# Tangshitao/Semi-supervised-Adaptive-Distillation

Measured on AMD Instinct MI355X. Metric: images/sec (student+teacher fwd + student bwd) R50-FPN distill, 1/2/4/8 MI355X, higher is better.
Workload: dtype f32

## Files before the change

include/ssad_kernels.h:

```cpp
#ifndef SSAD_KERNELS_H_
#define SSAD_KERNELS_H_

#include <stddef.h>
#include <stdint.h>

#ifdef __cplusplus
extern "C" {
#endif

#define SSAD_API __attribute__((visibility("default")))

#define SSAD_E_BADARG (-1)
#define SSAD_E_WORKSPACE (-2)
#define SSAD_MAX_LEVELS 8
#define SSAD_MAX_CONV_PROBLEMS 24
#define SSAD_MAX_POWSUM_INPUTS 8

typedef void* ssad_stream_t;


typedef struct {
  float gamma;
  float alpha;
  float beta;
// ... 223 lines not shown
    const double* cell_anchors, int levels, int A, int k_min, const int* field_sizes_host,
    const int* crop_h_host, const int* crop_w_host, const float* gt_boxes,
    const int* gt_classes, const int* gt_counts, int N, int Gmax, int num_classes,
    float positive_overlap, float negative_overlap, int* const* labels_out_host,
    float* const* locs_out_host, float* const* targets_out_host, int capacity,
    int* counts_out, float* fg_bg_out, void* workspace, size_t workspace_bytes,
    ssad_stream_t stream, int class_specific_bbox);


#define SSAD_IMAGE_BLOBS_MAX_BATCH 64
typedef struct ssad_image_norm {
  float div, mean[3], std[3];
  float* out;
} ssad_image_norm;
SSAD_API size_t ssad_image_blobs_workspace_bytes(int N, int Hb, int Wb);
SSAD_API int ssad_image_blobs(
    const unsigned char* src, size_t src_bytes, const long long* offset_host, const int* h_host,
    const int* w_host, const int* out_h_host, const int* out_w_host, const double* scale_host,
    const int* flipped_host, int N, int Hb, int Wb, const ssad_image_norm* norms_host, int n_norms,
    void* workspace, size_t workspace_bytes, ssad_stream_t stream);


SSAD_API int ssad_conv_out_size(int in, int kernel, int dilation, int pad_a, int pad_b, int stride);
SSAD_API int ssad_im2col(const float* x, int C, int H, int W, int kh, int kw, int dil_h, int dil_w,
                         int pad_t, int pad_l, int pad_b, int pad_r, int stride_h, int stride_w,
                         float* col, ssad_stream_t stream);
SSAD_API int ssad_im2col_batched(const float* x, int N, int C, int H, int W, int kernel, int stride,
                                 int pad, float* col, ssad_stream_t stream);
SSAD_API int ssad_col2im(const float* col, int C, int H, int W, int kh, int kw, int dil_h,
                         int dil_w, int pad_t, int pad_l, int pad_b, int pad_r, int stride_h,
                         int stride_w, float* x, ssad_stream_t stream);
SSAD_API int ssad_channel_sum(const float* dy, int N, int C, int HW, float* out, int accumulate,
                              ssad_stream_t stream);
SSAD_API int ssad_relu_grad_rowsum(const float* y, const float* dy, float* dx, float* rowsum, int N,
                                   int C, int HW, ssad_stream_t stream);
SSAD_API int ssad_conv1x1_bias_act(const float* x, const float* w, const float* bias,
                                   const float* residual, float* y, int N, int C, int P, int M,
                                   int relu, ssad_stream_t stream);
SSAD_API int ssad_conv1x1_bias_act2(const float* x, int C1, const float* x2, int C2, const float* w,
                                    const float* bias, const float* residual, float* y, int N, int P,
                                    int M, int relu, ssad_stream_t stream);
#define SSAD_GEMM_RELU 1
#define SSAD_GEMM_ACCUMULATE 8
typedef struct ssad_gemm_conv {
  const float* a;
  const float* x;
  float* y;
  const float* bias;
  const float* residual;
  const float* mask;
  int lda, N, K, P, M, flags;
} ssad_gemm_conv;
SSAD_API int ssad_conv1x1_gemm(const ssad_gemm_conv* desc_host, ssad_stream_t stream);
SSAD_API size_t ssad_conv1x1_gemm_split_workspace_bytes(const ssad_gemm_conv* desc_host);
SSAD_API int ssad_conv1x1_gemm_split(const ssad_gemm_conv* desc_host, void* workspace, size_t workspace_bytes,
                                     ssad_stream_t stream);
SSAD_API int ssad_conv1x1_gemm_split_amax(const ssad_gemm_conv* desc_host, const float* packed_a, const unsigned* x_amax,
                                          unsigned* y_amax_out, void* workspace, size_t workspace_bytes,
                                          ssad_stream_t stream);
typedef struct ssad_gemm_pack_entry {
  const float* a;
  float* dst;
  int lda, K, M;
} ssad_gemm_pack_entry;
SSAD_API size_t ssad_gemm_split_filter_floats(int K, int M);
SSAD_API int ssad_gemm_split_pack_filters(const ssad_gemm_pack_entry* entries_host, int n_entries, ssad_stream_t stream);
SSAD_API int ssad_conv_implicit_gemm(const ssad_gemm_conv* d, int C, int H, int W, int kernel, int stride, int pad,
                                     ssad_stream_t stream);
SSAD_API size_t ssad_conv_implicit_gemm_workspace_bytes(int N, int M, int C, int H, int W, int kernel, int stride,
                                                        int pad);
SSAD_API int ssad_conv_implicit_gemm_ws(const ssad_gemm_conv* d, int C, int H, int W, int kernel, int stride, int pad,
                                        void* workspace, size_t workspace_bytes, ssad_stream_t stream);
SSAD_API size_t ssad_conv_kxk_wgrad_workspace_bytes(int N, int C, int H, int W, int M, int kernel, int stride,
                                                    int pad);
SSAD_API int ssad_conv_kxk_wgrad(const float* x, const float* dy, int N, int C, int H, int W, int M, int kernel,
                                 int stride, int pad, float* dw, int accumulate, void* workspace,
                                 size_t workspace_bytes, ssad_stream_t stream);
SSAD_API size_t ssad_conv_kxk_dgrad_workspace_bytes(int N, int C, int H, int W, int M, int kernel, int stride,
                                                    int pad);
SSAD_API int ssad_conv_kxk_dgrad(const float* w, const float* dy, int N, int C, int H, int W, int M, int kernel,
                                 int stride, int pad, float* dx, const float* mask, int accumulate, void* workspace,
                                 size_t workspace_bytes, ssad_stream_t stream);
SSAD_API int ssad_transpose_filter(const float* w, int M, int K, int ldm, float* wt, ssad_stream_t stream);
#define SSAD_MAX_TRANSPOSE_ENTRIES 64
typedef struct ssad_transpose_entry {
  const float* w;
  float* wt;
  int M, K, ldm;
  int reserved;
} ssad_transpose_entry;
SSAD_API int ssad_transpose_filters(const ssad_transpose_entry* entries_host, int n_entries, ssad_stream_t stream);
SSAD_API size_t ssad_conv1x1_wgrad_workspace_bytes(int N, int C, int P, int M);
SSAD_API int ssad_conv1x1_wgrad(const float* x, const float* dy, int N, int C, int P, int M, float* dw,
                                int accumulate, void* workspace, size_t workspace_bytes,
                                ssad_stream_t stream);
SSAD_API size_t ssad_conv1x1_wgrad_split_workspace_bytes(int N, int C, int P, int M);
SSAD_API int ssad_conv1x1_wgrad_split(const float* x, const float* dy, int N, int C, int P, int M, float* dw,
                                      int accumulate, void* workspace, size_t workspace_bytes,
                                      ssad_stream_t stream);
SSAD_API int ssad_conv1x1_wgrad_split_amax(const float* x, const float* dy, int N, int C, int P, int M, float* dw,
                                           int accumulate, void* workspace, size_t workspace_bytes,
                                           const unsigned* x_amax, const unsigned* dy_amax, ssad_stream_t stream);
SSAD_API int ssad_subsample(const float* x, int N, int C, int H, int W, int stride, float* y,
                            ssad_stream_t stream);
SSAD_API int ssad_subsample_grad(const float* dy, int N, int C, int H, int W, int stride, int accumulate,
                                 float* dx, ssad_stream_t stream);
// ... 277 lines not shown
```

semi-supervised-adaptive-distillation_amd/csrc/kernels/gemm_conv.hip:

```cpp
#include <hip/hip_runtime.h>
#include <stdint.h>
#include <stdlib.h>

#include "conv_internal.h"
#include "ssad_kernels.h"

namespace {

using ssad_dev::uniform_rsrc;
typedef float f32x16 __attribute__((ext_vector_type(16)));
typedef __attribute__((address_space(3))) void* lds_ptr;

constexpr int kThreads = 256;
constexpr unsigned kOob = 0x80000000u;
constexpr int BN = 128;
constexpr int BK = 16;
constexpr int NSTAGE = 3;

struct GemmArgs {
  const float* a;
  const float* x;
  float* y;
  const float* bias;
  const float* res;
  const float* mask;
  int lda, N, K, P, M, flags;
  int mtiles, ctiles;
  long long Q;
  int C, H, W, OW, ksize, stride, pad;
  int splits, per_split;
  float* part;
};

__device__ __forceinline__ float ldf(__amdgpu_buffer_rsrc_t rs, unsigned off) {
  return __builtin_bit_cast(float, __builtin_amdgcn_raw_buffer_load_b32(rs, off, 0, 0));
}
__device__ __forceinline__ void stf(float v, __amdgpu_buffer_rsrc_t rs, unsigned off) {
  __builtin_amdgcn_raw_buffer_store_b32(__builtin_bit_cast(unsigned, v), rs, off, 0, 0);
}

__device__ __forceinline__ int xcd_remap(int b, int total) {
  const int q = total >> 3, r = total & 7;
  const int xcd = b & 7, k = b >> 3;
  return (xcd < r ? xcd * (q + 1) : r * (q + 1) + (xcd - r) * q) + k;
}

template <int BM, bool IMPLICIT = false>
__global__ __launch_bounds__(kThreads, 3) void gemm_conv_nn_kernel(const GemmArgs g) {
  constexpr int TI = BM / 64;
  constexpr int A_STAGE = BK * BM;
  constexpr int B_STAGE = BK * BN;
  constexpr int STAGE = A_STAGE + B_STAGE;
  constexpr int A_ROW_LANES = BM / 4;
  constexpr int A_ROWS_PER_INSTR = 64 / A_ROW_LANES;
  constexpr int A_INSTR = BK / A_ROWS_PER_INSTR;
  constexpr int B_INSTR = BK / 2;
  constexpr int A_PER_WAVE = A_INSTR / 4;
  constexpr int B_PER_WAVE = IMPLICIT ? BK * (BN / 64) / 4 : B_INSTR / 4;
  constexpr int LOADS = A_PER_WAVE + B_PER_WAVE;
  __shared__ __attribute__((aligned(16))) float lds[NSTAGE * STAGE];

  const int tid = threadIdx.x, lane = tid & 63, wave = __builtin_amdgcn_readfirstlane(tid >> 6);
  const int wm = wave & 1, wn = wave >> 1;
  const int j = lane & 31, h = lane >> 5;
  const int ntiles = g.mtiles * g.ctiles;
  const int split = g.splits > 1 ? (int)blockIdx.x / ntiles : 0;
  const int tile = xcd_remap((int)blockIdx.x - split * ntiles, ntiles);
  const int mt = tile % g.mtiles, ct = tile / g.mtiles;
  const int m0 = mt * BM;
  const long long q0 = (long long)ct * BN;
  const int K = g.K, P = g.P;

  const __amdgpu_buffer_rsrc_t ars = uniform_rsrc(g.a, (unsigned)((long long)K * g.lda * 4));
  const __amdgpu_buffer_rsrc_t xrs = uniform_rsrc(
      g.x, IMPLICIT ? (unsigned)((long long)g.N * g.C * g.H * g.W * 4) : (unsigned)((long long)g.N * K * P * 4));

  const int a_row = lane / A_ROW_LANES, a_col = (lane % A_ROW_LANES) * 4;
  unsigned a_voff = (unsigned)((a_row * g.lda + m0 + a_col) * 4);
  if (m0 + a_col >= g.lda) a_voff = kOob;
  const long long qb = q0 + (lane & 31) * 4;
  unsigned b_voff = kOob;
  if (qb < g.Q) {
    const int n = (int)(qb / P), p = (int)(qb - (long long)n * P);
    b_voff = (unsigned)((((long long)n * K + h) * P + p) * 4);
  }
  int ioff[2] = {0, 0};
  unsigned ymask[2] = {0, 0}, xmask[2] = {0, 0};
  int s_c[4] = {0, 0, 0, 0}, s_ky[4] = {0, 0, 0, 0}, s_kx[4] = {0, 0, 0, 0};
  int d_c = 0, d_ky = 0, d_kx = 0;
  if (IMPLICIT) {
#pragma unroll
    for (int hf = 0; hf < 2; ++hf) {
      const long long qc = q0 + hf * 64 + lane;
      const bool ok = qc < g.Q;
      const int n = ok ? (int)(qc / P) : 0, pp = ok ? (int)(qc - (long long)n * P) : 0;
      const int iy0 = (pp / g.OW) * g.stride - g.pad, ix0 = (pp % g.OW) * g.stride - g.pad;
      ioff[hf] = ((n * g.C * g.H + iy0) * g.W + ix0) * 4;
      if (ok)
        for (int t = 0; t < g.ksize; ++t) {
          ymask[hf] |= (unsigned)((unsigned)(iy0 + t) < (unsigned)g.H) << t;
          xmask[hf] |= (unsigned)((unsigned)(ix0 + t) < (unsigned)g.W) << t;
        }
    }
    const int kk2 = g.ksize * g.ksize;
    const int row0 = (g.splits > 1 ? split * g.per_split : 0) * BK + wave * 4;
#pragma unroll
    for (int v = 0; v < 4; ++v) {
      const int row = row0 + v, c = row / kk2, r2 = row - c * kk2;
      s_c[v] = c; s_ky[v] = r2 / g.ksize; s_kx[v] = r2 - s_ky[v] * g.ksize;
    }
    d_c = BK / kk2;
    const int d_r = BK - d_c * kk2;
    d_ky = d_r / g.ksize; d_kx = d_r - d_ky * g.ksize;
  }
  auto issue = [&](int chunk, int buf) {
    const int k0 = chunk * BK;
    float* base = lds + buf * STAGE;
    const bool tail = k0 + BK > K;
#pragma unroll
    for (int u = 0; u < A_PER_WAVE; ++u) {
      const int ia = wave * A_PER_WAVE + u;
      const int row = k0 + ia * A_ROWS_PER_INSTR;
      unsigned vo = a_voff;
      if (tail) vo = (row + a_row < K) ? a_voff : kOob;
      __builtin_amdgcn_raw_ptr_buffer_load_lds(ars, (lds_ptr)(base + ia * 256), 16, vo, row * g.lda * 4, 0, 0);
    }
    if (IMPLICIT) {
#pragma unroll
      for (int u = 0; u < B_PER_WAVE; ++u) {
        const int ib = wave * B_PER_WAVE + u;
        const int rr = ib >> 1, hf = ib & 1, v = u >> 1;
        const int soff = ((s_c[v] * g.H + s_ky[v]) * g.W + s_kx[v]) * 4;
        const unsigned in = (ymask[hf] >> s_ky[v]) & (xmask[hf] >> s_kx[v]) & 1u;
        unsigned vo = in ? (unsigned)(ioff[hf] + soff) : kOob;
        if (tail) vo = (k0 + rr < K) ? vo : kOob;
        __builtin_amdgcn_raw_ptr_buffer_load_lds(xrs, (lds_ptr)(base + A_STAGE + rr * BN + hf * 64), 4, vo, 0, 0, 0);
      }
#pragma unroll
      for (int v = 0; v < 4; ++v) {
        s_kx[v] += d_kx;
        if (s_kx[v] >= g.ksize) { s_kx[v] -= g.ksize; ++s_ky[v]; }
        s_ky[v] += d_ky;
        if (s_ky[v] >= g.ksize) { s_ky[v] -= g.ksize; ++s_c[v]; }
        s_c[v] += d_c;
      }
    } else {
#pragma unroll
      for (int u = 0; u < B_PER_WAVE; ++u) {
        const int ib = wave * B_PER_WAVE + u;
        const int row = k0 + ib * 2;
        unsigned vo = b_voff;
        if (tail) vo = (row + h < K) ? b_voff : kOob;
        __builtin_amdgcn_raw_ptr_buffer_load_lds(xrs, (lds_ptr)(base + A_STAGE + ib * 256), 16, vo, row * P * 4, 0, 0);
      }
    }
  };

  f32x16 acc[TI][2];
#pragma unroll
  for (int i = 0; i < TI; ++i)
#pragma unroll
    for (int t = 0; t < 2; ++t)
#pragma unroll
      for (int r = 0; r < 16; ++r) acc[i][t][r] = 0.0f;

  int chunk0 = 0, chunks = (K + BK - 1) / BK;
  if (g.splits > 1) {
    chunk0 = split * g.per_split;
    chunks = chunks < chunk0 + g.per_split ? chunks : chunk0 + g.per_split;
  }
  issue(chunk0, 0);
  if (chunk0 + 1 < chunks) issue(chunk0 + 1, 1);
  const int a_rd = wm * (BM / 2) + j;
  const int b_rd = A_STAGE + wn * 64 + j;
  int buf = 0;
  for (int c = chunk0; c < chunks; ++c) {
    if (c + 1 < chunks) {
      asm volatile("s_waitcnt vmcnt(%0)" ::"n"(LOADS) : "memory");
    } else {
      asm volatile("s_waitcnt vmcnt(0)" ::: "memory");
    }
    __builtin_amdgcn_s_barrier();
    if (c + 2 < chunks) issue(c + 2, buf == 0 ? 2 : buf - 1);
    typedef const volatile __attribute__((address_space(3))) float* lds_cvf;
    const lds_cvf sa = (lds_cvf)(lds + buf * STAGE + a_rd + h * BM);
    const lds_cvf sb = (lds_cvf)(lds + buf * STAGE + b_rd + h * BN);
    float av[2][TI], bv[2][2];
#pragma unroll
    for (int i = 0; i < TI; ++i) av[0][i] = sa[i * 32];
#pragma unroll
    for (int t = 0; t < 2; ++t) bv[0][t] = sb[t * 32];
#pragma unroll
    for (int ks = 0; ks < BK / 2; ++ks) {
      const int cur = ks & 1, nxt = cur ^ 1;
      if (ks + 1 < BK / 2) {
        const int k = 2 * (ks + 1);
#pragma unroll
        for (int i = 0; i < TI; ++i) av[nxt][i] = sa[k * BM + i * 32];
#pragma unroll
        for (int t = 0; t < 2; ++t) bv[nxt][t] = sb[k * BN + t * 32];
      }
      __builtin_amdgcn_sched_barrier(0);
#pragma unroll
      for (int i = 0; i < TI; ++i)
#pragma unroll
        for (int t = 0; t < 2; ++t)
          acc[i][t] = __builtin_amdgcn_mfma_f32_32x32x2f32(av[cur][i], bv[cur][t], acc[i][t], 0, 0, 0);
      __builtin_amdgcn_sched_barrier(0);
    }
    if (++buf == NSTAGE) buf = 0;
  }

  const bool partial = g.splits > 1;
  const bool relu = !partial && (g.flags & SSAD_GEMM_RELU), accum = !partial && (g.flags & SSAD_GEMM_ACCUMULATE);
  const float* const gbias = partial ? nullptr : g.bias;
  const float* const gres = partial ? nullptr : g.res;
  const float* const gmask = partial ? nullptr : g.mask;
  const long long ybytes = (long long)g.N * g.M * P * 4;
  float* const yout = partial ? g.part + (long long)split * ((long long)g.N * g.M * P) : g.y;
  const __amdgpu_buffer_rsrc_t yrs = uniform_rsrc(yout, (unsigned)ybytes);
  const __amdgpu_buffer_rsrc_t rrs = uniform_rsrc(gres ? gres : yout, (unsigned)ybytes);
  const __amdgpu_buffer_rsrc_t krs = uniform_rsrc(gmask ? gmask : yout, (unsigned)ybytes);
#pragma unroll
  for (int i = 0; i < TI; ++i) {
    float bvv[16];
#pragma unroll
    for (int r = 0; r < 16; ++r) bvv[r] = 0.0f;
    if (gbias) {
#pragma unroll
      for (int r = 0; r < 16; ++r) {
        const int m = m0 + wm * (BM / 2) + i * 32 + (r & 3) + 8 * (r >> 2) + 4 * h;
        bvv[r] = gbias[m < g.M ? m : g.M - 1];
      }
    }
#pragma unroll
    for (int t = 0; t < 2; ++t) {
      const long long q = q0 + wn * 64 + t * 32 + j;
      long long col = -1;
      if (q < g.Q) {
        const int n = (int)(q / P), p = (int)(q - (long long)n * P);
        col = (long long)n * g.M * P + p;
      }
      unsigned off[16];
#pragma unroll
      for (int r = 0; r < 16; ++r) {
        const int m = m0 + wm * (BM / 2) + i * 32 + (r & 3) + 8 * (r >> 2) + 4 * h;
        off[r] = (col >= 0 && m < g.M) ? (unsigned)((col + (long long)m * P) * 4) : kOob;
      }
      f32x16 v = acc[i][t];
#pragma unroll
      for (int r = 0; r < 16; ++r) v[r] += bvv[r];
      if (gres) {
        float tmp[16];
#pragma unroll
        for (int r = 0; r < 16; ++r) tmp[r] = ldf(rrs, off[r]);
#pragma unroll
        for (int r = 0; r < 16; ++r) v[r] += tmp[r];
      }
      if (relu) {
#pragma unroll
        for (int r = 0; r < 16; ++r) v[r] = fmaxf(v[r], 0.0f);
      }
      if (gmask) {
        float tmp[16];
#pragma unroll
        for (int r = 0; r < 16; ++r) tmp[r] = ldf(krs, off[r]);
#pragma unroll
        for (int r = 0; r < 16; ++r) v[r] = tmp[r] > 0.0f ? v[r] : 0.0f;
      }
      if (accum) {
        float tmp[16];
#pragma unroll
        for (int r = 0; r < 16; ++r) tmp[r] = ldf(yrs, off[r]);
#pragma unroll
        for (int r = 0; r < 16; ++r) v[r] += tmp[r];
      }
#pragma unroll
      for (int r = 0; r < 16; ++r) stf(v[r], yrs, off[r]);
    }
  }
}

struct WgradArgs {
  const float* x;
  const float* dy;
  float* part;
  int N, C, P, M;
  int mtiles, ctiles;
  int chunks;
  int per_split;
  int splits;
  int xcd_group;
};

__global__ __launch_bounds__(kThreads, 3) void gemm_conv_nt_kernel(const WgradArgs g) {
  constexpr int TSTAGE = 128 * BK;
  constexpr int STAGE = 2 * TSTAGE;
  __shared__ __attribute__((aligned(16))) float lds[NSTAGE * STAGE];
  const int tid = threadIdx.x, lane = tid & 63, wave = __builtin_amdgcn_readfirstlane(tid >> 6);
  const int wm = wave & 1, wn = wave >> 1;
  const int j = lane & 31, h = lane >> 5;
  int v = (int)blockIdx.x;
  {
    const int G = (int)gridDim.x, xg = g.xcd_group;
    if (xg > 1 && (G & 7) == 0 && ((G >> 3) % xg) == 0) {
      const int r = v >> 3, x = v & 7;
      v = (r / xg) * (8 * xg) + x * xg + (r % xg);
    }
  }
  const int ntiles = g.mtiles * g.ctiles;
  const int split = v / ntiles, tile = v - split * ntiles;
  const int mt = tile % g.mtiles, ct = tile / g.mtiles;
  const int m0 = mt * 128, c0 = ct * 128;
  const int P = g.P;
  const int ch0 = split * g.per_split;
  const int ch1 = min(ch0 + g.per_split, g.chunks);
  const int nch = ch1 - ch0;

  const __amdgpu_buffer_rsrc_t yrs = uniform_rsrc(g.dy, (unsigned)((long long)g.N * g.M * P * 4));
  const __amdgpu_buffer_rsrc_t xrs = uniform_rsrc(g.x, (unsigned)((long long)g.N * g.C * P * 4));

  const int d_row = lane >> 2, d_slot = lane & 3;
  unsigned vy0[2], vx0[2];
#pragma unroll
  for (int u = 0; u < 2; ++u) {
    const int row = (wave * 2 + u) * 16 + d_row;
    const int piece = d_slot ^ ((row >> 2) & 3);
    vy0[u] = (m0 + row < g.M) ? (unsigned)((((long long)(m0 + row)) * P + piece * 4) * 4) : kOob;
    vx0[u] = (c0 + row < g.C) ? (unsigned)((((long long)(c0 + row)) * P + piece * 4) * 4) : kOob;
  }
  auto issue = [&](int chunk, int buf) {
// ... 153 lines not shown
  const unsigned r = blockIdx.x * 4 + (threadIdx.x >> 6);
  if (r >= rows) return;
  const unsigned pl = r / (unsigned)OH, oy = r - pl * (unsigned)OH;
  const float4* src = reinterpret_cast<const float4*>(x + ((size_t)pl * H + 2 * oy) * W);
  float2* dst = reinterpret_cast<float2*>(y + (size_t)r * OW);
  for (int j = threadIdx.x & 63; j < (OW >> 1); j += 64) {
    const float4 v = src[j];
    dst[j] = make_float2(v.x, v.z);
  }
}

__global__ __launch_bounds__(kThreads) void subsample2_grad_kernel(const float* __restrict__ dy, unsigned rows, int H,
                                                                   int W, int OH, int OW, int accumulate,
                                                                   float* __restrict__ dx) {
  const unsigned r = blockIdx.x * 4 + (threadIdx.x >> 6);
  if (r >= rows) return;
  const unsigned pl = r / (unsigned)H, yh = r - pl * (unsigned)H;
  const bool live = !(yh & 1) && (yh >> 1) < (unsigned)OH;
  const float2* src = reinterpret_cast<const float2*>(dy + ((size_t)pl * OH + (yh >> 1)) * OW);
  float4* dst = reinterpret_cast<float4*>(dx + (size_t)r * W);
  for (int j = threadIdx.x & 63; j < (W >> 2); j += 64) {
    float4 v = make_float4(0.0f, 0.0f, 0.0f, 0.0f);
    if (live) { const float2 d = src[j]; v.x = d.x; v.z = d.y; }
    if (accumulate) { const float4 o = dst[j]; v.x += o.x; v.y += o.y; v.z += o.z; v.w += o.w; }
    dst[j] = v;
  }
}

__global__ __launch_bounds__(kThreads) void splitk_reduce_kernel(const float* __restrict__ part, int splits, long long n,
                                                                 const float* __restrict__ bias,
                                                                 const float* __restrict__ res,
                                                                 const float* __restrict__ mask, int flags, int M, int P,
                                                                 float* __restrict__ y) {
  for (long long i = (long long)blockIdx.x * kThreads + threadIdx.x; i < n; i += (long long)gridDim.x * kThreads) {
    float v = 0.0f;
    for (int s = 0; s < splits; ++s) v += part[(long long)s * n + i];
    if (bias) v += bias[(int)((i / P) % M)];
    if (res) v += res[i];
    if (flags & SSAD_GEMM_RELU) v = fmaxf(v, 0.0f);
    if (mask) v = mask[i] > 0.0f ? v : 0.0f;
    if (flags & SSAD_GEMM_ACCUMULATE) v += y[i];
    y[i] = v;
  }
}

int pick_splits(int tiles, int chunks) {
  const int cus = ssad_cu_count();
  int s = (3 * cus + tiles - 1) / tiles;
  const int cap = chunks / 8 > 0 ? chunks / 8 : 1;
  if (s > cap) s = cap;
  if (s > 256) s = 256;
  if (s < 1) s = 1;
  return s;
}

}

extern "C" {

int ssad_conv1x1_gemm(const ssad_gemm_conv* d, ssad_stream_t stream) {
  if (!d || !d->a || !d->x || !d->y || d->N < 0 || d->K < 1 || d->P < 1 || d->M < 1) return SSAD_E_BADARG;
  if (d->lda < d->M || (d->lda & 3) || (d->P & 3)) return SSAD_E_BADARG;
  if (((uintptr_t)d->a | (uintptr_t)d->x) & 15) return SSAD_E_BADARG;
  if ((d->flags & SSAD_GEMM_ACCUMULATE) && (d->bias || d->residual)) return SSAD_E_BADARG;
  const long long Q = (long long)d->N * d->P;
  if (Q == 0) return 0;
  const long long big = (long long)d->N * (d->K > d->M ? d->K : d->M) * d->P * 4;
  if (big >= (1LL << 31) || (long long)d->K * d->lda * 4 >= (1LL << 31)) return SSAD_E_BADARG;
  GemmArgs g;
  g.a = d->a; g.x = d->x; g.y = d->y; g.bias = d->bias; g.res = d->residual; g.mask = d->mask;
  g.lda = d->lda; g.N = d->N; g.K = d->K; g.P = d->P; g.M = d->M; g.flags = d->flags;
  g.Q = Q;
  g.ctiles = (int)((Q + BN - 1) / BN);
  g.C = g.H = g.W = g.OW = g.ksize = g.stride = g.pad = 0;
  g.splits = 1; g.per_split = 0; g.part = nullptr;
  hipStream_t s = (hipStream_t)stream;
  const int cus = ssad_cu_count();
  const bool small = (long long)((d->M + 127) / 128) * g.ctiles < 6LL * cus;
  if (d->M <= 64 || small) {
    g.mtiles = (d->M + 63) / 64;
    hipLaunchKernelGGL(gemm_conv_nn_kernel<64>, dim3(g.mtiles * g.ctiles), dim3(kThreads), 0, s, g);
  } else {
    g.mtiles = (d->M + 127) / 128;
    hipLaunchKernelGGL(gemm_conv_nn_kernel<128>, dim3(g.mtiles * g.ctiles), dim3(kThreads), 0, s, g);
  }
  return (int)hipGetLastError();
}

static void implicit_split_plan(int M, long long Q, int K, int* splits, int* per_split) {
  const int mt = M <= 64 ? (M + 63) / 64 : (M + 127) / 128;
  const long long tiles = (long long)mt * ((Q + BN - 1) / BN);
  const int chunks = (K + BK - 1) / BK;
  static const int force = [] { const char* e = getenv("SSAD_IMPLICIT_SPLITS"); return e ? atoi(e) : 0; }();
  long long s = (4LL * ssad_cu_count() + tiles - 1) / tiles;
  if (s > chunks / 16) s = chunks / 16;
  if (force > 0) s = force;
  if (s > chunks) s = chunks;
  if (s < 1) s = 1;
  const int per = (int)((chunks + s - 1) / s);
  *per_split = per;
  *splits = (chunks + per - 1) / per;
}

size_t ssad_conv_implicit_gemm_workspace_bytes(int N, int M, int C, int H, int W, int kernel, int stride, int pad) {
  if (N < 1 || M < 1 || C < 1 || kernel < 1 || stride < 1 || pad < 0 || H + 2 * pad < kernel || W + 2 * pad < kernel)
    return 0;
  const int OH = (H + 2 * pad - kernel) / stride + 1, OW = (W + 2 * pad - kernel) / stride + 1;
  int splits, per;
  implicit_split_plan(M, (long long)N * OH * OW, C * kernel * kernel, &splits, &per);
  return splits > 1 ? (size_t)splits * N * M * OH * OW * sizeof(float) : 0;
}

int ssad_conv_implicit_gemm_ws(const ssad_gemm_conv* d, int C, int H, int W, int kernel, int stride, int pad,
                               void* workspace, size_t workspace_bytes, ssad_stream_t stream) {
  if (!d || !d->a || !d->x || !d->y || d->N < 0 || d->M < 1 || C < 1 || H < 1 || W < 1) return SSAD_E_BADARG;
  if (kernel < 1 || stride < 1 || pad < 0 || H + 2 * pad < kernel || W + 2 * pad < kernel) return SSAD_E_BADARG;
  if (kernel > 32) return SSAD_E_BADARG;
  const int OH = (H + 2 * pad - kernel) / stride + 1, OW = (W + 2 * pad - kernel) / stride + 1;
  const int K = C * kernel * kernel;
  if (d->K != K || d->P != OH * OW) return SSAD_E_BADARG;
  if (d->lda < d->M || (d->lda & 3)) return SSAD_E_BADARG;
  if ((uintptr_t)d->a & 15) return SSAD_E_BADARG;
  if ((d->flags & SSAD_GEMM_ACCUMULATE) && (d->bias || d->residual)) return SSAD_E_BADARG;
  const long long Q = (long long)d->N * d->P;
  if (Q == 0) return 0;
  if ((long long)d->N * C * H * W * 4 >= (1LL << 31) || (long long)d->N * d->M * d->P * 4 >= (1LL << 31) ||
      (long long)K * d->lda * 4 >= (1LL << 31))
    return SSAD_E_BADARG;
  {
    if (C == 3 && kernel == 7 && stride == 2 && pad == 3 && d->M == 64 && !d->bias && !d->residual &&
        !d->mask && d->flags == 0)
      return ssad_stem7x7s2_launch(d->x, d->a, d->lda, d->N, H, W, d->y, (hipStream_t)stream);
  }
  GemmArgs g;
  g.a = d->a; g.x = d->x; g.y = d->y; g.bias = d->bias; g.res = d->residual; g.mask = d->mask;
  g.lda = d->lda; g.N = d->N; g.K = K; g.P = d->P; g.M = d->M; g.flags = d->flags;
  g.Q = Q;
  g.ctiles = (int)((Q + BN - 1) / BN);
  g.C = C; g.H = H; g.W = W; g.OW = OW; g.ksize = kernel; g.stride = stride; g.pad = pad;
// ... 133 lines not shown
```

semi-supervised-adaptive-distillation_amd/kernels.py:

```python
import ctypes as C
import os

import torch

_HERE = os.path.dirname(os.path.abspath(__file__))
LIB_NAME = "libcaffe2_detectron_ops_hip.so"
LIB_PATH = os.path.join(_HERE, LIB_NAME)

MAX_LEVELS = 8
CONV_RELU = 1
CONV_MASK_AUX = 2
CONV_SIGMOID = 4
CONV_SPLIT_TAIL = 8
CONV_ACCUM_AUX = 32


class KernelError(RuntimeError):
    pass


class DistillParams(C.Structure):
    _fields_ = [("gamma", C.c_float), ("alpha", C.c_float), ("beta", C.c_float),
                ("num_classes", C.c_int), ("ignored_label", C.c_int),
                ("scale", C.c_float)]
# ... 158 lines not shown
    L.ssad_upsample_nearest_grad.argtypes = [vp, vp, i32, i32, i32, i32, i32, vp]
    L.ssad_max_pool3x3s2_bias_relu.argtypes = [vp, vp, i32, i32, i32, i32, i32, vp, vp]
    L.ssad_relu_grad_rowsum.argtypes = [vp, vp, vp, vp, i32, i32, i32, vp]
    L.ssad_conv1x1_bias_act.argtypes = [vp, vp, vp, vp, vp, i32, i32, i32, i32, i32, vp]
    L.ssad_conv1x1_bias_act2.argtypes = [vp, i32, vp, i32, vp, vp, vp, vp, i32, i32, i32, i32, vp]
    L.ssad_f16_pack_activations.argtypes = [vp, i32, i32, i32, i32, f32, vp, vp]
    L.ssad_f16_unpack_activations.argtypes = [vp, i32, i32, i32, i32, f32, vp, vp]
    L.ssad_f16_filter_halves.restype = sz
    L.ssad_f16_filter_halves.argtypes = [i32, i32]
    L.ssad_f16_pack_filter.argtypes = [vp, i32, i32, vp, vp, vp]
    L.ssad_conv3x3_forward_f16.argtypes = [vp, vp, vp, vp, i32, i32, i32, i32, i32, i32, vp, vp]
    L.ssad_conv3x3_forward_f16_levels.argtypes = [C.POINTER(F16Level), i32, vp, vp, i32, i32, i32, vp]
    L.ssad_conv3x3_wgrad_f16_workspace_bytes.restype = sz
    L.ssad_conv3x3_wgrad_f16_workspace_bytes.argtypes = [i32, i32, i32, i32, i32]
    L.ssad_conv3x3_wgrad_f16.argtypes = [vp, vp, i32, i32, i32, i32, i32, i32, f32, vp, vp, vp, sz, vp]
    L.ssad_conv3x3_wgrad_f16_levels_workspace_bytes.restype = sz
    L.ssad_conv3x3_wgrad_f16_levels_workspace_bytes.argtypes = [C.POINTER(F16WgradLevel), i32, i32, i32]
    L.ssad_conv3x3_wgrad_f16_levels.argtypes = [C.POINTER(F16WgradLevel), i32, i32, i32, i32, f32, vp, vp,
                                                vp, sz, vp]
    L.ssad_momentum_sgd_update.argtypes = [vp, vp, vp, vp, f32, f32, i32, i64, vp]
    L.ssad_momentum_sgd_flat.argtypes = [vp, vp, vp, vp, f32, f32, C.POINTER(SgdSegment), i32, vp, vp]
    L.ssad_check_finite.argtypes = [vp, i64, vp, vp]
    L.ssad_loss_scale_update.argtypes = [vp, vp, f32, f32, i32, f32, f32, vp]
    L.ssad_conv_wino_pack_filters.argtypes = [C.POINTER(PackEntry), i32, vp]
    L.ssad_conv_packed_filter_floats.restype = sz
    L.ssad_conv_packed_filter_floats.argtypes = [i32, i32]
    L.ssad_conv_pack_filter.argtypes = [vp, i32, i32, vp, vp, vp]
    L.ssad_conv3x3_forward.argtypes = [C.POINTER(ConvLevel), i32, vp, vp, i32, i32, i32, vp]
    L.ssad_conv_wino_filter_floats.restype = sz
    L.ssad_conv_wino_filter_floats.argtypes = [i32, i32]
    L.ssad_conv_wino_pack_filter.argtypes = [vp, i32, i32, vp, vp, vp]
    L.ssad_conv3x3_forward_wino.argtypes = [C.POINTER(ConvLevel), i32, vp, vp, i32, i32, i32, vp]
    L.ssad_conv3x3_forward_wino24.argtypes = [C.POINTER(ConvLevel), i32, vp, vp, i32, i32, i32, vp]
    L.ssad_conv_wino24_filter_floats.restype = sz
    L.ssad_conv_wino24_filter_floats.argtypes = [i32, i32]
    L.ssad_conv_wino24_pack_filters.argtypes = [C.POINTER(PackEntry), i32, vp]
    L.ssad_conv_split_filter_floats.restype = sz
    L.ssad_conv_split_filter_floats.argtypes = [i32, i32]
    L.ssad_conv_split_pack_filters.argtypes = [C.POINTER(PackEntry), i32, vp]
    L.ssad_conv3x3_split_workspace_bytes.restype = sz
    L.ssad_conv3x3_split_workspace_bytes.argtypes = [C.POINTER(ConvLevel), i32, i32]
    L.ssad_conv3x3_split_items.argtypes = [C.POINTER(ConvLevel), i32, i32]
    L.ssad_conv3x3_forward_split.argtypes = [C.POINTER(ConvLevel), i32, vp, vp, i32, i32, i32, vp, sz, vp, vp, vp]
    L.ssad_conv3x3_forward_wino_launches.argtypes = [C.POINTER(ConvLevel), i32]
    L.ssad_conv3x3_forward_wino_launches_for.argtypes = [C.POINTER(ConvLevel), i32, i32, i32, i32]
    L.ssad_conv_wino_split_tail.argtypes = [i32]
    L.ssad_conv3x3_wgrad_workspace_bytes.restype = sz
    L.ssad_conv3x3_wgrad_workspace_bytes.argtypes = [C.POINTER(ConvLevel), i32, i32, i32]
    L.ssad_conv3x3_wgrad.argtypes = [C.POINTER(ConvLevel), i32, vp, vp, i32, i32, i32, vp, sz, vp]
    L.ssad_conv3x3_wgrad_split_workspace_bytes.restype = sz
    L.ssad_conv3x3_wgrad_split_workspace_bytes.argtypes = [C.POINTER(ConvLevel), i32, i32, i32]
    L.ssad_conv3x3_wgrad_split.argtypes = [C.POINTER(ConvLevel), i32, vp, vp, i32, i32, i32, vp, sz, vp]
    L.ssad_conv1x1_gemm.argtypes = [C.POINTER(GemmConv), vp]
    L.ssad_conv1x1_gemm_split_workspace_bytes.restype = sz
    L.ssad_conv1x1_gemm_split_workspace_bytes.argtypes = [C.POINTER(GemmConv)]
    L.ssad_conv1x1_gemm_split.argtypes = [C.POINTER(GemmConv), vp, sz, vp]
    L.ssad_transpose_filter.argtypes = [vp, i32, i32, i32, vp, vp]
    L.ssad_conv1x1_wgrad_workspace_bytes.restype = sz
    L.ssad_conv1x1_wgrad_workspace_bytes.argtypes = [i32, i32, i32, i32]
    L.ssad_conv1x1_wgrad.argtypes = [vp, vp, i32, i32, i32, i32, vp, i32, vp, sz, vp]
    L.ssad_gemm_split_filter_floats.restype = sz
    L.ssad_gemm_split_filter_floats.argtypes = [i32, i32]
    L.ssad_gemm_split_pack_filters.argtypes = [C.POINTER(GemmPackEntry), i32, vp]
    L.ssad_conv1x1_gemm_split_amax.argtypes = [vp, vp, vp, vp, vp, sz, vp]
    L.ssad_split_absmax.argtypes = [vp, C.c_longlong, vp, vp]
    L.ssad_split_absmax_levels.argtypes = [C.POINTER(ConvLevel), i32, i32, i32, vp, vp]
    L.ssad_conv3x3_wgrad_split_amax.argtypes = [C.POINTER(ConvLevel), i32, vp, vp, i32, i32, i32, vp, sz, vp, vp, vp]
    L.ssad_conv1x1_wgrad_split_amax.argtypes = [vp, vp, i32, i32, i32, i32, vp, i32, vp, sz, vp, vp, vp]
    L.ssad_conv1x1_wgrad_split_workspace_bytes.restype = sz
    L.ssad_conv1x1_wgrad_split_workspace_bytes.argtypes = [i32, i32, i32, i32]
    L.ssad_conv1x1_wgrad_split.argtypes = [vp, vp, i32, i32, i32, i32, vp, i32, vp, sz, vp]
    L.ssad_subsample.argtypes = [vp, i32, i32, i32, i32, i32, vp, vp]
    L.ssad_subsample_grad.argtypes = [vp, i32, i32, i32, i32, i32, i32, vp, vp]
    L.ssad_conv_implicit_gemm.argtypes = [C.POINTER(GemmConv), i32, i32, i32, i32, i32, i32, vp]
    L.ssad_transpose_filters.argtypes = [C.POINTER(TransposeEntry), i32, vp]
    L.ssad_f16_pack_filters.argtypes = [C.POINTER(F16PackEntry), i32, vp]
    L.ssad_conv_implicit_gemm_workspace_bytes.restype = sz
    L.ssad_conv_implicit_gemm_workspace_bytes.argtypes = [i32] * 8
    L.ssad_conv_implicit_gemm_ws.argtypes = [C.POINTER(GemmConv), i32, i32, i32, i32, i32, i32, vp, sz, vp]
    L.ssad_conv_kxk_wgrad_workspace_bytes.restype = sz
    L.ssad_conv_kxk_wgrad_workspace_bytes.argtypes = [i32] * 8
    L.ssad_conv_kxk_wgrad.argtypes = [vp, vp, i32, i32, i32, i32, i32, i32, i32, i32, vp, i32, vp, sz, vp]
    L.ssad_conv_kxk_dgrad_workspace_bytes.restype = sz
    L.ssad_conv_kxk_dgrad_workspace_bytes.argtypes = [i32] * 8
    L.ssad_conv_kxk_dgrad.argtypes = [vp, vp, i32, i32, i32, i32, i32, i32, i32, i32, vp, vp, i32, vp, sz, vp]
    L.ssad_grouped_conv3x3_forward.argtypes = [vp, vp, vp, i32, i32, i32, i32, i32, i32, i32, vp, vp]
    L.ssad_grouped_conv3x3_filter_floats.argtypes = [i32, i32]
    L.ssad_grouped_conv3x3_filter_floats.restype = C.c_longlong
    L.ssad_grouped_conv3x3_pack_filter.argtypes = [vp, i32, i32, vp, vp]
    L.ssad_grouped_conv3x3_dgrad_filter_floats.argtypes = [i32, i32]
    L.ssad_grouped_conv3x3_dgrad_filter_floats.restype = C.c_longlong
    L.ssad_grouped_conv3x3_pack_filter_dgrad.argtypes = [vp, i32, i32, vp, vp]
    L.ssad_grouped_conv3x3_dgrad.argtypes = [vp, vp, vp, i32, i32, i32, i32, i32, i32, vp, vp]
    L.ssad_grouped_conv3x3_wgrad_workspace_bytes.restype = sz
    L.ssad_grouped_conv3x3_wgrad_workspace_bytes.argtypes = [i32] * 6
    L.ssad_grouped_conv3x3_wgrad.argtypes = [vp, vp, i32, i32, i32, i32, i32, i32, vp, vp, sz, vp]
    L.ssad_grouped_conv3x3_pack_filters.argtypes = [C.POINTER(GroupedPackEntry), i32, vp]
    L.ssad_conv1x1_f16.argtypes = [C.POINTER(PwF16), vp]
    L.ssad_pw_f16_filter_halves.restype = sz
    L.ssad_pw_f16_filter_halves.argtypes = [i32, i32]
    L.ssad_pw_f16_pack_filter.argtypes = [vp, i32, i32, vp, vp, vp]
    L.ssad_conv1x1_wgrad_f16_workspace_bytes.restype = sz
    L.ssad_conv1x1_wgrad_f16_workspace_bytes.argtypes = [i32, i32, i32, i32, i32]
    L.ssad_conv1x1_wgrad_f16.argtypes = [vp, vp, i32, i32, i32, i32, i32, i32, f32, vp, vp, vp, vp, sz, vp]
    L.ssad_f16_elementwise.argtypes = [i32, vp, vp, vp, i32, i32, i32, i32, i32, i32, vp]
    L.ssad_f16_subsample.argtypes = [vp, i32, i32, i32, i32, i32, vp, vp]
# ... 1125 lines not shown
```

Baseline: 252.1.

## Specialize pointwise GEMM epilogue at compile time and prefetch epilogue operands

Adds compile-time epilogue variants of the 1x1 conv GEMM kernel, chosen from which of bias, residual, mask and accumulate are present. These variants precompute output offsets with 32-bit math and take row masks from readfirstlane. They prefetch residual, mask and old-output values during the last K chunk and software-pipeline those loads across output blocks. The aim is to cut runtime branching and 64-bit index arithmetic in the epilogue, and to hide epilogue load latency behind the final MFMAs. In exchange it adds ablation macros, an env override, a tile-rows query API, more template instances, and higher register pressure.

Result: no change. 253.0 (median of 6 runs) (+0.4%).

```diff
diff --git a/include/ssad_kernels.h b/include/ssad_kernels.h
--- a/include/ssad_kernels.h
+++ b/include/ssad_kernels.h
@@ -299,6 +299,7 @@
   int lda, N, K, P, M, flags;
 } ssad_gemm_conv;
 SSAD_API int ssad_conv1x1_gemm(const ssad_gemm_conv* desc_host, ssad_stream_t stream);
+SSAD_API int ssad_conv1x1_gemm_tile_rows(const ssad_gemm_conv* desc_host);
 SSAD_API size_t ssad_conv1x1_gemm_split_workspace_bytes(const ssad_gemm_conv* desc_host);
 SSAD_API int ssad_conv1x1_gemm_split(const ssad_gemm_conv* desc_host, void* workspace, size_t workspace_bytes,
                                      ssad_stream_t stream);
diff --git a/semi-supervised-adaptive-distillation_amd/csrc/kernels/gemm_conv.hip b/semi-supervised-adaptive-distillation_amd/csrc/kernels/gemm_conv.hip
--- a/semi-supervised-adaptive-distillation_amd/csrc/kernels/gemm_conv.hip
+++ b/semi-supervised-adaptive-distillation_amd/csrc/kernels/gemm_conv.hip
@@ -16,6 +16,10 @@
 constexpr int BN = 128;
 constexpr int BK = 16;
 constexpr int NSTAGE = 3;
+#ifndef GCONV_ABLATE
+#define GCONV_ABLATE 0
+#endif
+constexpr int kEpiBias = 1, kEpiRes = 2, kEpiMask = 4, kEpiAcc = 8, kEpiRuntime = 16;
 
 struct GemmArgs {
   const float* a;
@@ -39,14 +43,23 @@
   __builtin_amdgcn_raw_buffer_store_b32(__builtin_bit_cast(unsigned, v), rs, off, 0, 0);
 }
 
+__device__ __forceinline__ float ldfs(__amdgpu_buffer_rsrc_t rs, unsigned off, int soff) {
+  return __builtin_bit_cast(float, __builtin_amdgcn_raw_buffer_load_b32(rs, off, soff, 0));
+}
+__device__ __forceinline__ void stfs(float v, __amdgpu_buffer_rsrc_t rs, unsigned off, int soff) {
+  __builtin_amdgcn_raw_buffer_store_b32(__builtin_bit_cast(unsigned, v), rs, off, soff, 0);
+}
+
 __device__ __forceinline__ int xcd_remap(int b, int total) {
   const int q = total >> 3, r = total & 7;
   const int xcd = b & 7, k = b >> 3;
   return (xcd < r ? xcd * (q + 1) : r * (q + 1) + (xcd - r) * q) + k;
 }
 
-template <int BM, bool IMPLICIT = false>
+template <int BM, bool IMPLICIT = false, int EPI = kEpiRuntime>
 __global__ __launch_bounds__(kThreads, 3) void gemm_conv_nn_kernel(const GemmArgs g) {
+  constexpr bool FAST = EPI != kEpiRuntime;
+  static_assert(!(FAST && IMPLICIT), "the implicit GEMM reads its options at run time");
   constexpr int TI = BM / 64;
   constexpr int A_STAGE = BK * BM;
   constexpr int B_STAGE = BK * BN;
@@ -80,7 +93,13 @@
   if (m0 + a_col >= g.lda) a_voff = kOob;
   const long long qb = q0 + (lane & 31) * 4;
   unsigned b_voff = kOob;
-  if (qb < g.Q) {
+  if constexpr (FAST) {
+    const unsigned qu = (unsigned)qb;
+    if (qu < (unsigned)g.Q) {
+      const unsigned n = qu / (unsigned)P, p = qu - n * (unsigned)P;
+      b_voff = ((n * (unsigned)K + (unsigned)h) * (unsigned)P + p) * 4u;
+    }
+  } else if (qb < g.Q) {
     const int n = (int)(qb / P), p = (int)(qb - (long long)n * P);
     b_voff = (unsigned)((((long long)n * K + h) * P + p) * 4);
   }
@@ -169,12 +188,56 @@
     chunk0 = split * g.per_split;
     chunks = chunks < chunk0 + g.per_split ? chunks : chunk0 + g.per_split;
   }
+  constexpr int NB = 2 * TI;
+  const int mw = m0 + wm * (BM / 2);
+  const int P4 = __builtin_amdgcn_readfirstlane(P * 4);
+  unsigned cvo[2] = {kOob, kOob}, gm[TI][4];
+  float bs[TI][16], rs[2][16], mk[2][16], old[2][16];
+  __amdgpu_buffer_rsrc_t yrs_f = ars, rrs_f = ars, krs_f = ars;
+  if constexpr (FAST) {
+#pragma unroll
+    for (int t = 0; t < 2; ++t) {
+      const unsigned q = (unsigned)q0 + wn * 64 + t * 32 + j;
+      if (q < (unsigned)g.Q) {
+        const unsigned n = q / (unsigned)P, p = q - n * (unsigned)P;
+        cvo[t] = ((n * (unsigned)g.M + (unsigned)(mw + 4 * h)) * (unsigned)P + p) * 4u;
+      }
+    }
+#pragma unroll
+    for (int i = 0; i < TI; ++i)
+#pragma unroll
+      for (int gr = 0; gr < 4; ++gr) gm[i][gr] = __builtin_amdgcn_readfirstlane(mw + i * 32 + 8 * gr < g.M ? 0u : kOob);
+    const unsigned ybytes = (unsigned)((long long)g.N * g.M * P * 4);
+    yrs_f = uniform_rsrc(g.y, ybytes);
+    if constexpr (EPI & kEpiRes) rrs_f = uniform_rsrc(g.res, ybytes);
+    if constexpr (EPI & kEpiMask) krs_f = uniform_rsrc(g.mask, ybytes);
+    if constexpr (EPI & kEpiBias) {
+      const __amdgpu_buffer_rsrc_t brs = uniform_rsrc(g.bias, (unsigned)g.M * 4u);
+#pragma unroll
+      for (int i = 0; i < TI; ++i)
+#pragma unroll
+        for (int r = 0; r < 16; ++r)
+          bs[i][r] = ldfs(brs, (unsigned)(mw + 4 * h) * 4u | gm[i][r >> 2], (i * 32 + 8 * (r >> 2) + (r & 3)) * 4);
+    }
+  }
+  auto issue_ops = [&](int b, int s) {
+    const int i = b >> 1, t = b & 1;
+#pragma unroll
+    for (int r = 0; r < 16; ++r) {
+      const unsigned vo = cvo[t] | gm[i][r >> 2];
+      const int so = (i * 32 + 8 * (r >> 2) + (r & 3)) * P4;
+      if constexpr (EPI & kEpiRes) rs[s][r] = ldfs(rrs_f, vo, so);
+      if constexpr (EPI & kEpiMask) mk[s][r] = ldfs(krs_f, vo, so);
+      if constexpr (EPI & kEpiAcc) old[s][r] = ldfs(yrs_f, vo, so);
+    }
+  };
+
   issue(chunk0, 0);
   if (chunk0 + 1 < chunks) issue(chunk0 + 1, 1);
   const int a_rd = wm * (BM / 2) + j;
   const int b_rd = A_STAGE + wn * 64 + j;
   int buf = 0;
-  for (int c = chunk0; c < chunks; ++c) {
+  auto run_chunk = [&](int c, auto before_mfmas) {
     if (c + 1 < chunks) {
       asm volatile("s_waitcnt vmcnt(%0)" ::"n"(LOADS) : "memory");
     } else {
@@ -190,6 +253,7 @@
     for (int i = 0; i < TI; ++i) av[0][i] = sa[i * 32];
 #pragma unroll
     for (int t = 0; t < 2; ++t) bv[0][t] = sb[t * 32];
+    before_mfmas();
 #pragma unroll
     for (int ks = 0; ks < BK / 2; ++ks) {
       const int cur = ks & 1, nxt = cur ^ 1;
@@ -204,18 +268,64 @@
 #pragma unroll
       for (int i = 0; i < TI; ++i)
 #pragma unroll
-        for (int t = 0; t < 2; ++t)
-          acc[i][t] = __builtin_amdgcn_mfma_f32_32x32x2f32(av[cur][i], bv[cur][t], acc[i][t], 0, 0, 0);
+        for (int t = 0; t < 2; ++t) {
+          if (GCONV_ABLATE & 4)
+            acc[i][t][0] += av[cur][i] + bv[cur][t];
+          else
+            acc[i][t] = __builtin_amdgcn_mfma_f32_32x32x2f32(av[cur][i], bv[cur][t], acc[i][t], 0, 0, 0);
+        }
       __builtin_amdgcn_sched_barrier(0);
     }
     if (++buf == NSTAGE) buf = 0;
-  }
+  };
+
+  if constexpr (FAST) {
+    for (int c = chunk0; c < chunks - 1; ++c) run_chunk(c, [] {});
+    run_chunk(chunks - 1, [&] {
+      __builtin_amdgcn_sched_barrier(0);
+      issue_ops(0, 0);
+      __builtin_amdgcn_sched_barrier(0);
+    });
+    const bool relu = g.flags & SSAD_GEMM_RELU;
+#pragma unroll
+    for (int b = 0; b < NB; ++b) {
+      const int i = b >> 1, t = b & 1, s = b & 1;
+      __builtin_amdgcn_sched_barrier(0);
+      if (b + 1 < NB) issue_ops(b + 1, (b + 1) & 1);
+      __builtin_amdgcn_sched_barrier(0);
+      f32x16 v = acc[i][t];
+#pragma unroll
+      for (int r = 0; r < 16; ++r) v[r] += (EPI & kEpiBias) ? bs[i][r] : 0.0f;
+      if constexpr (EPI & kEpiRes) {
+#pragma unroll
+        for (int r = 0; r < 16; ++r) v[r] += rs[s][r];
+      }
+      if (relu) {
+#pragma unroll
+        for (int r = 0; r < 16; ++r) v[r] = fmaxf(v[r], 0.0f);
+      }
+      if constexpr (EPI & kEpiMask) {
+#pragma unroll
+        for (int r = 0; r < 16; ++r) v[r] = mk[s][r] > 0.0f ? v[r] : 0.0f;
+      }
+      if constexpr (EPI & kEpiAcc) {
+#pragma unroll
+        for (int r = 0; r < 16; ++r) v[r] += old[s][r];
+      }
+#pragma unroll
+      for (int r = 0; r < 16; ++r)
+        stfs(v[r], yrs_f, cvo[t] | gm[i][r >> 2], (i * 32 + 8 * (r >> 2) + (r & 3)) * P4);
+    }
+    return;
+  }
+  for (int c = chunk0; c < chunks; ++c) run_chunk(c, [] {});
 
   const bool partial = g.splits > 1;
-  const bool relu = !partial && (g.flags & SSAD_GEMM_RELU), accum = !partial && (g.flags & SSAD_GEMM_ACCUMULATE);
+  const bool relu = !partial && (g.flags & SSAD_GEMM_RELU);
+  const bool accum = !partial && !(GCONV_ABLATE & 1) && (g.flags & SSAD_GEMM_ACCUMULATE);
   const float* const gbias = partial ? nullptr : g.bias;
-  const float* const gres = partial ? nullptr : g.res;
-  const float* const gmask = partial ? nullptr : g.mask;
+  const float* const gres = partial || (GCONV_ABLATE & 1) ? nullptr : g.res;
+  const float* const gmask = partial || (GCONV_ABLATE & 1) ? nullptr : g.mask;
   const long long ybytes = (long long)g.N * g.M * P * 4;
   float* const yout = partial ? g.part + (long long)split * ((long long)g.N * g.M * P) : g.y;
   const __amdgpu_buffer_rsrc_t yrs = uniform_rsrc(yout, (unsigned)ybytes);
@@ -246,6 +356,7 @@
       for (int r = 0; r < 16; ++r) {
         const int m = m0 + wm * (BM / 2) + i * 32 + (r & 3) + 8 * (r >> 2) + 4 * h;
         off[r] = (col >= 0 && m < g.M) ? (unsigned)((col + (long long)m * P) * 4) : kOob;
+        if (GCONV_ABLATE & 8) off[r] = ((((unsigned)blockIdx.x * (2 * TI) + i * 2 + t) * 16 + r) * kThreads + tid) * 4u;
       }
       f32x16 v = acc[i][t];
 #pragma unroll
@@ -276,7 +387,7 @@
         for (int r = 0; r < 16; ++r) v[r] += tmp[r];
       }
 #pragma unroll
-      for (int r = 0; r < 16; ++r) stf(v[r], yrs, off[r]);
+      for (int r = 0; r < 16; ++r) stf(v[r], yrs, (GCONV_ABLATE & 2) ? off[r] | kOob : off[r]);
     }
   }
 }
@@ -536,6 +647,34 @@
   if (s > 256) s = 256;
   if (s < 1) s = 1;
   return s;
+}
+
+int pointwise_tile_rows(int M, long long ctiles) {
+  const bool small = (long long)((M + 127) / 128) * ctiles < 6LL * ssad_cu_count();
+  return (M <= 64 || small) ? 64 : 128;
+}
+
+bool conv_generic_forced() {
+  const char* e = getenv("SSAD_GEMM_CONV_GENERIC");
+  return e && *e && atoi(e) != 0;
+}
+
+template <int BM>
+void launch_pointwise(const GemmArgs& g, int epi, hipStream_t s) {
+  const dim3 grid(g.mtiles * g.ctiles), block(kThreads);
+  switch (epi) {
+#define SSAD_GCONV_FORM(E) \
+  case (E): hipLaunchKernelGGL((gemm_conv_nn_kernel<BM, false, (E)>), grid, block, 0, s, g); break;
+    SSAD_GCONV_FORM(0)
+    SSAD_GCONV_FORM(kEpiBias)
+    SSAD_GCONV_FORM(kEpiBias | kEpiRes)
+    SSAD_GCONV_FORM(kEpiMask)
+    SSAD_GCONV_FORM(kEpiAcc)
+    SSAD_GCONV_FORM(kEpiMask | kEpiAcc)
+    SSAD_GCONV_FORM(kEpiRes | kEpiMask)
+#undef SSAD_GCONV_FORM
+    default: hipLaunchKernelGGL((gemm_conv_nn_kernel<BM, false, kEpiRuntime>), grid, block, 0, s, g);
+  }
 }
 
 }
@@ -559,16 +698,22 @@
   g.C = g.H = g.W = g.OW = g.ksize = g.stride = g.pad = 0;
   g.splits = 1; g.per_split = 0; g.part = nullptr;
   hipStream_t s = (hipStream_t)stream;
-  const int cus = ssad_cu_count();
-  const bool small = (long long)((d->M + 127) / 128) * g.ctiles < 6LL * cus;
-  if (d->M <= 64 || small) {
+  int epi = (d->bias ? kEpiBias : 0) | (d->residual ? kEpiRes : 0) | (d->mask ? kEpiMask : 0) |
+            ((d->flags & SSAD_GEMM_ACCUMULATE) ? kEpiAcc : 0);
+  if ((d->M & 7) || conv_generic_forced()) epi = kEpiRuntime;
+  if (pointwise_tile_rows(d->M, g.ctiles) == 64) {
     g.mtiles = (d->M + 63) / 64;
-    hipLaunchKernelGGL(gemm_conv_nn_kernel<64>, dim3(g.mtiles * g.ctiles), dim3(kThreads), 0, s, g);
+    launch_pointwise<64>(g, epi, s);
   } else {
     g.mtiles = (d->M + 127) / 128;
-    hipLaunchKernelGGL(gemm_conv_nn_kernel<128>, dim3(g.mtiles * g.ctiles), dim3(kThreads), 0, s, g);
+    launch_pointwise<128>(g, epi, s);
   }
   return (int)hipGetLastError();
+}
+
+int ssad_conv1x1_gemm_tile_rows(const ssad_gemm_conv* d) {
+  if (!d || d->N < 0 || d->P < 1 || d->M < 1) return 0;
+  return pointwise_tile_rows(d->M, ((long long)d->N * d->P + BN - 1) / BN);
 }
 
 static void implicit_split_plan(int M, long long Q, int K, int* splits, int* per_split) {
diff --git a/semi-supervised-adaptive-distillation_amd/kernels.py b/semi-supervised-adaptive-distillation_amd/kernels.py
--- a/semi-supervised-adaptive-distillation_amd/kernels.py
+++ b/semi-supervised-adaptive-distillation_amd/kernels.py
@@ -234,6 +234,7 @@
     L.ssad_conv3x3_wgrad_split_workspace_bytes.argtypes = [C.POINTER(ConvLevel), i32, i32, i32]
     L.ssad_conv3x3_wgrad_split.argtypes = [C.POINTER(ConvLevel), i32, vp, vp, i32, i32, i32, vp, sz, vp]
     L.ssad_conv1x1_gemm.argtypes = [C.POINTER(GemmConv), vp]
+    L.ssad_conv1x1_gemm_tile_rows.argtypes = [C.POINTER(GemmConv)]
     L.ssad_conv1x1_gemm_split_workspace_bytes.restype = sz
     L.ssad_conv1x1_gemm_split_workspace_bytes.argtypes = [C.POINTER(GemmConv)]
     L.ssad_conv1x1_gemm_split.argtypes = [C.POINTER(GemmConv), vp, sz, vp]
```
